# pashtari/factorizer

Hardware: AMD Instinct MI355X
Metric: volumes/sec fwd+bwd, Swin Factorizer 128^3 (higher is better)
Workload: dtype f32

## Files before the change

### factorizer_amd/_native.py

```python
from __future__ import annotations

import ctypes
import os
import threading

import torch

_HERE = os.path.dirname(os.path.abspath(__file__))
LIB_PATH = os.environ.get("FZ_LIB_PATH") or os.path.join(_HERE, "libfactorizer_hip.so")

FZ_OK = 0
FZ_E_UNSUPPORTED = -2
ABI_VERSION = 7
SOLVER_ID = {"mu": 0, "hals": 1, "cd": 2, "smu": 3}
STORE_F32, STORE_BF16 = 0, 1
PRODUCTS_DEFAULT, PRODUCTS_SPLIT_BF16, PRODUCTS_FP32_MFMA = 0, 1, 2
_products = threading.local()


def products() -> int:
    return getattr(_products, "value", PRODUCTS_DEFAULT)


class use_products:
# ... 184 lines not shown
    "fz_gcorr_wgrad": ([_vp] * 4 + [_i] * 11 + [_vp], _i),
    "fz_gcorr_act": ([_vp] * 5 + [_i] * 11 + [_f, _i, _vp], _i),
    "fz_gcorr_wgrad_act": ([_vp] * 4 + [_i] * 12 + [_vp], _i),
    "fz_gcorr_mu_bwd": ([_vp] * 8 + [_i] * 11 + [_f, _i, _vp], _i),
    "fz_gnmf_supported": ([_i, _i64, _i, _i, _i], _i),
    "fz_gnmf_workspace_bytes": ([_i64, _i, _i64, _i, _i, _i], _i64),
    "fz_gnmf_launches": ([_i, _i, _i], _i),
    "fz_gnmf_fwd": ([_vp] * 6 + [_i64, _i, _i64, _i, _i, _i, _f, _vp, _vp], _i),
    "fz_gnmf_bwd": ([_vp] * 7 + [_i64, _i, _i64, _i, _i, _i, _i, _f, _vp, _vp], _i),
    "fz_nmf_cf_supported": ([_i] * 11, _i),
    "fz_nmf_cf_fwd": ([_vp] * 4 + [_i] * 5 + [_c.POINTER(_i)] + [_i] * 5 + [_f, _i, _vp], _i),
    "fz_nmf_cf_bwd": ([_vp] * 5 + [_i] * 5 + [_c.POINTER(_i)] + [_i] * 7 + [_f, _i, _vp], _i),
    "fz_nmf_cf_factors_supported": ([_i] * 12 + [_c.POINTER(_i)], _i),
    "fz_nmf_cf_fwd_store_factors": ([_vp] * 5 + [_i] * 5 + [_c.POINTER(_i)] + [_i] * 3 + [_f, _i, _vp], _i),
    "fz_nmf_cf_fwd_from_factors": ([_vp] * 6 + [_i] * 5 + [_c.POINTER(_i)] * 2 + [_i] * 4 + [_f, _i, _vp], _i),
    "fz_nmf_cf_bwd_factors_supported": ([_i] * 14 + [_c.POINTER(_i)], _i),
    "fz_nmf_cf_bwd_store_factors": ([_vp] * 5 + [_i] * 5 + [_c.POINTER(_i)] + [_i] * 3 + [_f, _i, _vp], _i),
    "fz_nmf_cf_bwd_from_factors": ([_vp] * 6 + [_i] * 5 + [_c.POINTER(_i)] * 2 + [_i] * 3 + [_f, _i, _vp], _i),
    "fz_nmf_pcf_supported": ([_i] * 11, _i),
    "fz_nmf_pcf_fwd": ([_vp] * 4 + [_i] * 8 + [_c.POINTER(_i)] + [_i] * 5 + [_f, _i, _vp], _i),
    "fz_nmf_pcf_bwd": ([_vp] * 5 + [_i] * 8 + [_c.POINTER(_i)] + [_i] * 7 + [_f, _i, _vp], _i),
    "fz_nmf_pcf_bwd_prefers_separate": ([_i] * 4, _i),
    "fz_act_add": ([_vp, _vp, _i64, _i, _vp], _i),
    "fz_mlp_pre_supported": ([_i, _i, _i64, _i], _i),
    "fz_mlp_drop_supported": ([_i, _i, _i64, _i], _i),
    "fz_mlp_chain_drop": ([_c.POINTER(MlpDesc), _c.POINTER(MlpDropout), _vp], _i),
    "fz_conv3_prologue_supported": ([_i] * 4, _i),
    "fz_conv3_fwd2": ([_vp] * 4 + [_i] * 8 + [_c.POINTER(BlockPrologue), _vp], _i),
    "fz_upcat2": ([_vp, _vp, _vp, _i, _vp, _vp, _vp] + [_i] * 7 + [_c.POINTER(BlockPrologue), _vp], _i),
    "fz_gemm": ([_c.POINTER(GemmDesc), _vp], _i),
    "fz_gemm_bx_enable": ([_i], _i),
    "fz_gemm_lnbwd_partials": ([_c.POINTER(GemmDesc)], _i64),
    "fz_reduce_rows": ([_vp, _i64, _i, _vp, _vp, _vp], _i),
    "fz_adamw_step": ([_vp, _vp, _vp, _vp, _i64, _f, _f, _f, _f, _f, _i, _f, _vp], _i),
    "fz_sw_gather": ([_vp, _vp] + [_i] * 10 + [_vp], _i),
    "fz_sw_accumulate": ([_vp] * 6 + [_f] + [_i] * 10 + [_vp], _i),
    "fz_sw_finalize": ([_vp, _vp, _i, _i64, _vp], _i),
    "fz_sw_gather2": ([_vp, _vp] + [_i] * 11 + [_vp], _i),
    "fz_sw_accumulate2": ([_vp] * 6 + [_f] + [_i] * 11 + [_vp], _i),
    "fz_sw_finalize2": ([_vp, _vp, _vp, _i, _i64, _i, _vp], _i),
    "fz_mlp_supported": ([_i, _i, _i64], _i),
    "fz_mlp_partials": ([_i, _i64], _i64),
    "fz_mlp_wgrad_rows": ([_i, _i64], _i),
    "fz_gemm_dw_rows": ([_i, _i64], _i),
    "fz_gemm_dw_workspace_bytes": ([_i, _i64], _i64),
    "fz_gemm_dw": ([_c.POINTER(GemmDwDesc), _vp], _i),
    "fz_mlp_wgrad_workspace_bytes": ([_i, _i64], _i64),
    "fz_mlp_chain": ([_c.POINTER(MlpDesc), _vp], _i),
    "fz_head_bwd_rows": ([], _i),
    "fz_head_bwd_workspace_bytes": ([], _i64),
    "fz_head_bwd": ([_vp, _vp, _vp, _vp, _vp, _i, _i, _i, _i64, _i, _vp], _i),
    "fz_head_fwd": ([_vp, _vp, _vp, _vp, _i, _i, _i, _i64, _i, _vp], _i),
    "fz_upcat_supported": ([_i] * 5, _i),
    "fz_upcat_compose": ([_vp, _vp, _i, _vp, _vp, _vp, _vp, _vp, _i, _i, _i, _vp], _i),
    "fz_upcat_wgrads": ([_vp, _vp, _vp, _i, _vp, _vp, _vp, _vp, _i, _vp, _i, _i, _i, _vp], _i),
    "fz_upcat": ([_vp, _vp, _vp, _i, _vp, _vp, _vp] + [_i] * 7 + [_vp], _i),
    "fz_upcat_bwd_supported": ([_i] * 6, _i),
    "fz_upcat_bwd_workspace_bytes": ([_i] * 4, _i64),
    "fz_upcat_bwd": ([_vp, _vp, _vp, _vp, _i, _vp, _vp, _vp, _vp, _vp, _i, _vp, _vp] + [_i] * 7 + [_vp], _i),
    "fz_wgrad": ([_c.POINTER(WgradDesc), _vp, _vp], _i),
    "fz_wgrad_group": ([_c.POINTER(_c.POINTER(WgradDesc)), _c.POINTER(_vp), _i, _vp], _i),
    "fz_wgrad_workspace_bytes": ([_c.POINTER(WgradDesc)], _i64),
    "fz_conv3_fwd": ([_vp] * 4 + [_i] * 8 + [_vp], _i),
    "fz_conv3_wgrad_chunks": ([_i] * 4, _i),
    "fz_conv3_wgrad_partials": ([_vp] * 4 + [_i] * 8 + [_vp], _i),
    "fz_chunk_reduce": ([_vp, _i, _i64, _vp, _i, _vp], _i),
    "fz_chunk_reduce_ld": ([_vp, _i, _i64, _i64, _vp, _i, _vp], _i),
    "fz_finish_defer": ([_i], _i),
    "fz_finish_pending": ([], _i),
    "fz_finish_flush": ([_vp], _i),
    "fz_finish_flush_all": ([_vp], _i),
    "fz_dice_bce_chunks": ([_i64], _i),
    "fz_dice_bce_sums": ([_vp, _vp, _vp, _i, _i64, _vp], _i),
    "fz_dice_bce_grad": ([_vp, _vp, _vp, _vp, _i, _i64, _f, _f, _vp, _vp], _i),
    "fz_dice_ce_sums": ([_vp, _vp, _vp, _i, _i, _i64, _vp], _i),
    "fz_dice_ce_grad": ([_vp, _vp, _vp, _vp, _i, _i, _i64, _f, _f, _vp, _vp], _i),
    "fz_dice_ce_finish": ([_vp, _i, _i, _i64, _f, _vp, _vp, _vp], _i),
    "fz_dice_bce_ds_sums": ([_vp, _vp, _vp, _i] + [_i] * 6 + [_i, _vp], _i),
    "fz_dice_bce_ds_grad": ([_vp, _vp, _vp, _vp, _i] + [_i] * 6 + [_i, _f, _f, _vp, _vp], _i),
    "fz_dice_ce_ds_sums": ([_vp, _vp, _vp, _i, _i] + [_i] * 6 + [_i, _vp], _i),
    "fz_dice_ce_ds_grad": ([_vp, _vp, _vp, _vp, _i, _i] + [_i] * 6 + [_i, _f, _f, _vp, _vp], _i),
    "fz_rowsum_chunks": ([_i64], _i),
    "fz_rowsum": ([_vp, _vp, _vp, _i, _i, _i64, _i, _vp], _i),
    "fz_ln_fwd": ([_vp] * 5 + [_i, _i, _i64, _f, _i, _vp], _i),
    "fz_ln_bwd": ([_vp] * 8 + [_i, _i, _i64, _i, _vp], _i),
    "fz_ln_bwd_workspace_bytes": ([_i], _i64),
    "fz_ln_bwd_workspace_bytes2": ([_i, _i, _i64], _i64),
    "fz_dropout_bits_words": ([_i, _i, _i64], _i64),
    "fz_dropout_keep_bits": ([_vp, _i, _i, _i, _i64, _f, _vp, _vp], _i),
    "fz_dropout_apply": ([_i, _vp, _f, _vp, _vp, _vp, _i, _i, _i64, _i, _vp], _i),
    "fz_seg_counts_chunks": ([_i64], _i),
    "fz_seg_counts_workspace_bytes": ([_i, _i64], _i64),
    "fz_seg_counts": ([_vp, _i, _vp, _i, _f, _vp, _vp, _vp, _i, _i64, _vp], _i),
    "fz_mask_edges": ([_vp, _vp, _vp, _i, _i, _i, _i, _i, _vp], _i),
    "fz_edge_min_dist2_splits": ([_i64, _i64], _i),
    "fz_edge_min_dist2_workspace_bytes": ([_i64, _i64], _i64),
    "fz_edge_min_dist2": ([_vp, _i64, _vp, _i64, _f, _f, _f, _vp, _vp, _vp], _i),
    "fz_aug_record_floats": ([], _i),
    "fz_aug_resample": ([_vp, _vp, _i, _i, _vp, _vp, _i, _vp, _vp, _vp] + [_i] * 6 + [_vp], _i),
    "fz_aug_smooth": ([_vp, _vp, _i, _i, _vp, _vp] + [_i] * 6 + [_vp], _i),
    "fz_aug_noise_field": ([_vp, _vp, _i, _i, _i64, _vp], _i),
    "fz_aug_source_words": ([], _i),
    "fz_aug_crop_resample": ([_vp, _vp, _i, _i, _vp, _i, _vp, _vp, _vp] + [_i] * 6 + [_vp], _i),
    "fz_vol_kind_ok": ([_i, _i], _i),
    "fz_vol_bbox": ([_vp, _i, _i, _i, _i, _i, _i, _vp, _vp], _i),
    "fz_vol_workspace_bytes": ([_i, _c.POINTER(VolGeom)], _i64),
# ... 18 lines not shown
```

### factorizer_amd/blocks.py

```python
from __future__ import annotations

import os

import torch
from torch import nn

from . import functional as Fn
from . import pointwise as PW
from .layers import MLP, LayerNorm, Linear
from .matricize import Matricize, SWMatricize
from .nmf import NMF, MatrixFactorization, RandomInit
from .utils import partialize


def _env_int(name, default):
    v = os.environ.get(name)
    if v is None:
        return default
    try:
        return int(v, 0)
    except ValueError:
        raise ValueError(f"{name}={v!r}: expected an integer") from None


# ... 37 lines not shown
        self.mlp = MLP(channels, ratio=mlp_ratio, dropout=dropout)

    def _fusable(self, x) -> bool:
        f, m = self.fact, self.mlp
        if not (x.is_cuda and x.numel() and x.dtype in (torch.float32, torch.bfloat16) and PW._vox(x) % 4 == 0
                and x.shape[1] % 2 == 0):
            return False
        if any(p.dtype != torch.float32 for p in self.parameters()):
            return False
        if not (isinstance(self.norm1, LayerNorm) and isinstance(self.norm2, LayerNorm)
                and self.norm1.norm.elementwise_affine and self.norm2.norm.elementwise_affine
                and self.norm1.norm.bias is not None and self.norm2.norm.bias is not None):
            return False
        if not (isinstance(f.act, nn.ReLU) and isinstance(f.in_proj, Linear) and isinstance(f.out_proj, Linear)):
            return False
        blk = m.block
        if not (len(blk) == 5 and isinstance(blk[1], nn.GELU) and blk[1].approximate == "none"
                and blk[0].linear.weight.shape[0] % 2 == 0):
            return False
        drops = (f.dropout, blk[2], blk[4])
        if self.training and any(d.p > 0 for d in drops):
            return all(type(d) is nn.Dropout and 0 <= d.p < 1 for d in drops)
        return True

    def _dropout_ps(self):
        ps = (float(self.fact.dropout.p), float(self.mlp.block[2].p), float(self.mlp.block[4].p))
        return ps if self.training and any(p > 0 for p in ps) else None

    def _modular_native_cfg(self, x) -> bool:
        f = self.fact
        mf = f.factorize
        if not (isinstance(f.reshape, SWMatricize) and isinstance(mf, MatrixFactorization)):
            return False
        t_like = x.new_empty((1, *f.reshape.output_size[1:]))
        return mf._native_solver(t_like) is not None and not mf._wide and len(f.reshape.geometry.spatial) <= 3

    def _core_cfg(self):
        f = self.fact
        mf = f.factorize
        if not (isinstance(f.reshape, SWMatricize) and isinstance(mf, MatrixFactorization)):
            return None
        sid = getattr(mf.solver, "native_id", None)
        if sid is None or not isinstance(mf.init, RandomInit) or mf.solver.factor != (0, 1) or mf.verbose:
            return None
        G = min(max(mf.num_grad_steps, 0), mf.num_iters)
        geo = f.reshape.geometry
        if tuple(mf.size) != (8, geo.P) or not Fn.nmf_core_supported(geo, mf.rank, mf.num_iters, G):
            return None
        return G, sid

    def prologue_params(self, like):
        f, blk = self.fact, self.mlp.block
        n1 = self.norm1.norm
        if not (like.is_cuda and like.shape[1] == 32 and self._fusable(like) and self._core_cfg() is not None
                and f.in_proj.linear.bias is None and blk[0].linear.bias is not None and blk[3].linear.bias is not None
                and f.out_proj.linear.bias is not None and f.in_proj.linear.weight.dtype == torch.float32
                and n1.weight is not None and n1.bias is not None
                and not (self.norm1._forward_hooks or f.in_proj._forward_hooks or f._forward_hooks)):
            return None
        return n1.weight, n1.bias, n1.eps, f.in_proj.linear.weight

    def forward(self, x):
        if self._fusable(x):
            f, blk = self.fact, self.mlp.block
            n1, n2 = self.norm1.norm, self.norm2.norm
            core = self._core_cfg()
            mf = f.factorize
            nat = core is not None or self._modular_native_cfg(x)
            drop = self._dropout_ps()
            one_node = nat and f.in_proj.linear.bias is None and blk[0].linear.bias is not None \
                and blk[3].linear.bias is not None and f.out_proj.linear.bias is not None
            if one_node:
                if core is not None:
                    G, sid = core
                else:
                    G, sid = min(max(mf.num_grad_steps, 0), mf.num_iters), mf.solver.native_id
                cfg = dict(geo=f.reshape.geometry, T=mf.num_iters, G=G, solver=sid, nmf_eps=mf.solver.eps,
                           eps1=n1.eps, eps2=n2.eps, core=core is not None)
                if drop is not None:
                    cfg["drop"] = drop
                args = (x, n1.weight, n1.bias, f.in_proj.linear.weight, mf.init.u0, mf.init.v0,
                        f.out_proj.linear.weight, f.out_proj.linear.bias, n2.weight, n2.bias,
                        blk[0].linear.weight, blk[0].linear.bias, blk[3].linear.weight, blk[3].linear.bias, cfg)
                pre = PW.BlockPrologue.take(x) if core is not None else None
                t_pre, st_pre = pre if pre is not None else (None, None)
                slot = PW.head_fusion_slot()
                if slot is not None and slot.block is self and core is not None and drop is None:
                    hw, hb = slot.head_params
                    C, Hd = x.shape[1], blk[0].linear.weight.shape[0]
                    if PW.block_head_fusable(C, Hd, x[0, 0].numel(), hw, x):
                        y, raw = PW.FactorizerBlockFn.apply(*args, hw, hb, t_pre, st_pre)
                        slot.logits = PW.HeadOfBlockFn.apply(y, hw, hb, raw)
                        return y
                return PW.FactorizerBlockFn.apply(*args, None, None, t_pre, st_pre)
            if drop is None:
                return self._per_layer(x)
        x = x + self.fact(self.norm1(x))
        x = x + self.mlp(self.norm2(x))
        return x

    def _per_layer(self, x):
        f, blk = self.fact, self.mlp.block
        n1, n2 = self.norm1.norm, self.norm2.norm
        t = PW.ln_linear(x, n1.weight, n1.bias, n1.eps, f.in_proj.linear.weight, f.in_proj.linear.bias, "relu")
        a = f.reshape.inverse_forward(f.factorize(f.reshape(t)))
        x = PW.act_linear_res(a, f.out_proj.linear.weight, f.out_proj.linear.bias, x, "none")
        z = PW.ln_linear(x, n2.weight, n2.bias, n2.eps, blk[0].linear.weight, blk[0].linear.bias, "none")
# ... 66 lines not shown
```

### factorizer_amd/csrc/upcat.hip

```cpp
#include "gemm_bx.h"
#include "finish.h"

namespace fz {

template <typename AT>
struct UpcatArgsT {
  const AT* skip;
  const AT* deep;
  const float* wa;
  const float* wbt;
  const float* bias;
  AT* out;
  int lda;
  int B, D, H, W;
  BlockPrologueArgs pro;
};

#ifndef UPCAT_WAVES
#define UPCAT_WAVES 4
#endif
#define UPCAT_THREADS (UPCAT_WAVES * 64)
template <typename AT, bool PRO = false>
__global__ __launch_bounds__(UPCAT_THREADS, 1) void upcat_bx_kernel(UpcatArgsT<AT> p, unsigned ntiles) {
  constexpr int C = 32, CD = 64;
// ... 177 lines not shown
  if (tile + tstep < ntiles) fetch(tile + tstep, xsB, xdB);
  for (; tile < ntiles; tile += 2 * tstep) {
    run(tile, xsA, xdA);
    if (tile + tstep < ntiles) run(tile + tstep, xsB, xdB);
  }
}

__global__ __launch_bounds__(256) void upcat_compose_kernel(const float* __restrict__ w_t, const float* __restrict__ w_b, int ldb,
                                                            const float* __restrict__ b_t, const float* __restrict__ b_ad,
                                                            float* __restrict__ wc, float* __restrict__ wbt,
                                                            float* __restrict__ bias, int Cd, int O, int M) {
  const int k = blockIdx.x;
  if (k == Cd) {
    if (bias == nullptr) return;
    for (int m = threadIdx.x; m < M; m += 256) {
      float t = b_ad != nullptr ? b_ad[m] : 0.f;
      if (b_t != nullptr)
        for (int c = 0; c < O; ++c) t += w_b[(int64_t)m * ldb + c] * b_t[c];
      bias[m] = t;
    }
    return;
  }
  const float* wk = w_t + (int64_t)k * O * 8;
  for (int i = threadIdx.x; i < M * 8; i += 256) {
    const int m = i >> 3, t = i & 7;
    float acc = 0.f;
    for (int c = 0; c < O; ++c) acc += wk[c * 8 + t] * w_b[(int64_t)m * ldb + c];
    if (wc != nullptr) wc[((int64_t)k * M + m) * 8 + t] = acc;
    if (wbt != nullptr) wbt[((int64_t)t * M + m) * Cd + k] = acc;
  }
}


}

using namespace fz;

extern "C" int fz_upcat_compose(const float* w_t, const float* w_b, int ldb, const float* b_t, const float* b_ad, float* wc, float* wbt,
                                float* bias, int Cd, int O, int M, fz_stream_t stream) {
  if (!w_t || !w_b || (!wc && !wbt && !bias) || Cd < 1 || O < 1 || M < 1 || ldb < O) return fail(FZ_E_ARG, "fz_upcat_compose: bad arguments");
  hipLaunchKernelGGL(upcat_compose_kernel, dim3((unsigned)(Cd + 1)), dim3(256), 0, (hipStream_t)stream, w_t, w_b, ldb, b_t, b_ad, wc, wbt,
                     bias, Cd, O, M);
  FZ_LAUNCH_CHECK();
  return FZ_OK;
}

extern "C" int fz_upcat_wgrads(const float* gt, const float* w_t, const float* w_b, int ldb, const float* gb_ad, const float* b_t,
                               float* gw_t, float* gw_b, int ldg, float* gb_t, int Cd, int O, int M, fz_stream_t stream) {
  if (!gt || !w_t || !w_b || !gb_ad || !gw_t || !gw_b || Cd < 1 || O < 1 || M < 1 || ldb < O || ldg < O)
    return fail(FZ_E_ARG, "fz_upcat_wgrads: bad arguments");
  FinishJob fj = finish_job(FK_UPCAT, fin_upcat_blocks(Cd, O, M), 1);
  fj.u.up = FinUpcat{gt, w_t, w_b, gb_ad, b_t, gw_t, gw_b, gb_t, ldb, ldg, Cd, O, M};
  return finish_run(&fj, 1, (hipStream_t)stream);
}

extern "C" int fz_upcat_supported(int C, int Cd, int D, int H, int W) {
  return C == 32 && Cd == 64 && D >= 1 && H >= 1 && W >= 1 && (2 * W) % 64 == 0 && ((int64_t)2 * H * 2 * W) % 256 == 0 &&
         (int64_t)64 * D * H * W * 8 * 4 < ((int64_t)1 << 31);
}

template <typename AT>
static int upcat_launch(const void* skip, const void* deep, const float* wa, int lda, const float* wbt, const float* bias, void* out,
                        int B, int D, int H, int W, const fz_block_prologue* pro, fz_stream_t stream) {
  UpcatArgsT<AT> a;
  a.pro = BlockPrologueArgs{};
  if (pro) a.pro = BlockPrologueArgs{pro->ln_g, pro->ln_b, pro->ln_eps, pro->w, pro->t, pro->stats};
  a.skip = (const AT*)skip; a.deep = (const AT*)deep; a.wa = wa; a.wbt = wbt; a.bias = bias; a.out = (AT*)out;
  a.lda = lda; a.B = B; a.D = D; a.H = H; a.W = W;
  const int64_t ntiles = (int64_t)8 * D * H * W / 64 * B;
  if (ntiles >= ((int64_t)1 << 30)) return fail(FZ_E_ARG, "fz_upcat: more than 2^30 wave tiles (32-bit tile arithmetic)");
  constexpr int lds = (2 + 8 * 4) * 3 * 64 * 16 + 2 * 3 * 64 * 16 + 32 * 4;
  const int64_t wgs = (ntiles + UPCAT_WAVES - 1) / UPCAT_WAVES;
  if (pro) {
    auto kern = upcat_bx_kernel<AT, true>;
    FZ_HIP_OK(hipFuncSetAttribute(reinterpret_cast<const void*>(kern), hipFuncAttributeMaxDynamicSharedMemorySize, lds));
    hipLaunchKernelGGL(kern, dim3((unsigned)(wgs < 256 ? wgs : 256)), dim3(UPCAT_THREADS), lds, (hipStream_t)stream, a, (unsigned)ntiles);
    FZ_LAUNCH_CHECK();
    return FZ_OK;
  }
  auto kern = upcat_bx_kernel<AT>;
  FZ_HIP_OK(hipFuncSetAttribute(reinterpret_cast<const void*>(kern), hipFuncAttributeMaxDynamicSharedMemorySize, lds));
  hipLaunchKernelGGL(kern, dim3((unsigned)(wgs < 256 ? wgs : 256)), dim3(UPCAT_THREADS), lds, (hipStream_t)stream, a, (unsigned)ntiles);
  FZ_LAUNCH_CHECK();
  return FZ_OK;
}

extern "C" int fz_upcat2(const void* skip, const void* deep, const float* wa, int lda, const float* wbt, const float* bias, void* out,
                         int B, int C, int Cd, int D, int H, int W, int act_dtype, const fz_block_prologue* pro, fz_stream_t stream) {
  if (!skip || !deep || !wa || !wbt || !out) return fail(FZ_E_ARG, "fz_upcat: null pointer");
  if (pro && (!pro->ln_g || !pro->ln_b || !pro->w || !pro->t || !pro->stats)) return fail(FZ_E_ARG, "fz_upcat2: incomplete block prologue");
  if (!fz_upcat_supported(C, Cd, D, H, W) || lda < C) return fail(FZ_E_UNSUPPORTED, "fz_upcat: needs C = 32, 64 deep channels, 2W % 64 == 0, 4HW % 256 == 0");
  if (B <= 0) return B == 0 ? FZ_OK : fail(FZ_E_SHAPE, "fz_upcat: negative batch");
  if (act_dtype == FZ_STORE_F32) return upcat_launch<float>(skip, deep, wa, lda, wbt, bias, out, B, D, H, W, pro, stream);
  if (act_dtype == FZ_STORE_BF16) return upcat_launch<bf16>(skip, deep, wa, lda, wbt, bias, out, B, D, H, W, pro, stream);
  return fail(FZ_E_ARG, "fz_upcat: act_dtype must be FZ_STORE_F32 or FZ_STORE_BF16");
}

extern "C" int fz_upcat(const void* skip, const void* deep, const float* wa, int lda, const float* wbt, const float* bias, void* out,
                        int B, int C, int Cd, int D, int H, int W, int act_dtype, fz_stream_t stream) {
  return fz_upcat2(skip, deep, wa, lda, wbt, bias, out, B, C, Cd, D, H, W, act_dtype, nullptr, stream);
}
```

### factorizer_amd/pointwise.py

```python
from __future__ import annotations

import collections
import ctypes
import os
import threading as _threading
import weakref

import torch
import torch.nn.functional as F

from . import _native as N
from . import gradbuf as _GB
from . import functional as Fn

ACT = {"none": 0, "relu": 1, "gelu": 2}
LOAD_PLAIN, LOAD_S2D, LOAD_K3, LOAD_S2D_2D, LOAD_K3_2D = 0, 1, 2, 3, 4
EPI_PLAIN, EPI_D2S, EPI_D2S_2D = 0, 1, 3
QL_S2D_2D, QL_K3_2D = LOAD_S2D_2D, LOAD_K3_2D
_D2S_FINE = {EPI_D2S: 8, EPI_D2S_2D: 4}


def _p(t):
    return None if t is None else t.data_ptr()

# ... 995 lines not shown
    y = torch.matmul(weight.reshape(weight.shape[0], weight.shape[1]), x.reshape(B, C, _vox(x)))
    if bias is not None:
        y = y + bias.view(1, -1, 1)
    return y.reshape(B, weight.shape[0], *x.shape[2:])


def layernorm_cf(x, weight, bias, eps):
    if weight is not None and bias is not None and _native_ok(x, weight, bias):
        return LayerNormFn.apply(x, weight, bias, eps)
    _warn_composed("LayerNorm", x, weight, bias)
    y = F.layer_norm(x.movedim(1, -1), (x.shape[1],), weight, bias, eps)
    return y.movedim(-1, 1).contiguous()


def mlp_cf(x, w1, b1, w2, b2):
    if _native_ok(x, w1, b1, w2, b2) and w1.shape[1] % 2 == 0 and w2.shape[1] % 2 == 0:
        z = LinearFn.apply(x, w1, b1)
        return ActLinearResFn.apply(z, w2, b2, None, "gelu")
    _warn_composed("MLP", x, w1, b1, w2, b2)
    return linear_cf(F.gelu(linear_cf(x, w1, b1)), w2, b2)


def ln_linear(x, ln_w, ln_b, eps, w, b, act="none"):
    if _native_ok(x, ln_w, ln_b, w, b) and w.shape[1] % 2 == 0:
        return LNLinearFn.apply(x, ln_w, ln_b, eps, w, b, act)
    _warn_composed("LayerNorm+Linear", x, ln_w, ln_b, w, b)
    y = linear_cf(layernorm_cf(x, ln_w, ln_b, eps), w, b)
    return torch.relu(y) if act != "none" else y


def act_linear_res(z, w, b, res, act="none"):
    if _native_ok(z, w, b, res) and w.shape[1] % 2 == 0:
        return ActLinearResFn.apply(z, w, b, res, act)
    _warn_composed("Linear+residual", z, w, b, res)
    y = linear_cf(F.gelu(z) if act == "gelu" else z, w, b)
    return y if res is None else res + y


class UpCatLinearFn(torch.autograd.Function):

    _fz_acts = (0, 1, 6)

    @staticmethod
    @_fwd
    def forward(ctx, skip, deep, w_t, b_t, w_ad, b_ad, pro=None):
        skip, deep = skip.contiguous(), deep.contiguous()
        B, Cd, D, H, W = deep.shape
        O = w_t.shape[1]
        V = D * H * W
        C1 = skip.shape[1]
        M = w_ad.shape[0]
        w2 = w_ad.reshape(M, C1 + O)
        y = torch.empty((B, M, *skip.shape[2:]), dtype=skip.dtype, device=skip.device)
        if (M == 32 and C1 == 32 and O == 32 and _UPCAT_FWD and N.lib().fz_upcat_supported(C1, Cd, D, H, W)):
            w_b = w2[:, C1:]
            wbt = torch.empty((8, M, Cd), dtype=torch.float32, device=skip.device)
            bias = torch.empty(M, dtype=torch.float32, device=skip.device) if (b_t is not None or b_ad is not None) else None
            with torch.cuda.device(skip.device):
                N.check(N.lib().fz_upcat_compose(w_t.data_ptr(), w_b.data_ptr(), C1 + O, _p(b_t), _p(b_ad), None, wbt.data_ptr(),
                                                 _p(bias), Cd, O, M, N.stream_ptr(skip)), "fz_upcat_compose")
            es = skip.element_size()
            bp = None
            if pro is not None:
                ln_w, ln_b, eps, w_in = pro
                t_pro = torch.empty_like(y)
                st_pro = torch.empty((B, 2, 8 * V), dtype=torch.float32, device=skip.device)
                bp = N.BlockPrologue(ln_w.data_ptr(), ln_b.data_ptr(), float(eps), w_in.data_ptr(), t_pro.data_ptr(), st_pro.data_ptr())
            with torch.cuda.device(skip.device):
                rc = Fn._timed(f"upcat_{Cd}->{M}" + ("_ln_linear" if bp is not None else ""),
                               es * (skip.numel() + deep.numel() + y.numel() * (2 if bp is not None else 1)),
                               lambda: N.lib().fz_upcat2(skip.data_ptr(), deep.data_ptr(), w2.data_ptr(), C1 + O, wbt.data_ptr(),
                                                         _p(bias), y.data_ptr(), B, C1, Cd, D, H, W, N.act_dtype(skip),
                                                         ctypes.byref(bp) if bp is not None else None, N.stream_ptr(skip)),
                               cols=B * 8 * V, flops=2 * B * 8 * V * M * (C1 + Cd))
            N.check(rc, "fz_upcat")
        elif pro is not None:
            raise RuntimeError("UpCatLinearFn: a block prologue needs the one-pass forward (callers check upcat_prologue_ok)")
        else:
            up = torch.empty((B, O, 2 * D, 2 * H, 2 * W), dtype=deep.dtype, device=deep.device)
            _gemm([deep], w_t, up, B=B, Cin=Cd, Vin=V, M=8 * O, K=Cd, Ncol=V, w_t=True, ldw=8 * O, bias=b_t,
                  epilogue=EPI_D2S, Ho=H, Wo=W, name="tconv_k2s2")
            _gemm([skip, up], w2, y, B=B, Cin=C1 + O, Vin=8 * V, M=M, K=C1 + O, Ncol=8 * V, bias=b_ad, c0=C1, name="cat_linear")
        ctx.save_for_backward(skip, deep, w_t, w2, b_t)
        ctx.has_bt, ctx.has_bad, ctx.wshape = b_t is not None, b_ad is not None, w_ad.shape
        ctx.npro = 0 if pro is None else 1
        if pro is not None:
            ctx.mark_non_differentiable(t_pro, st_pro)
            ctx.set_materialize_grads(False)
            return y, t_pro, st_pro
        return y

    @staticmethod
    def _backward_three(ctx, g, skip, deep, w2, wc, gw_ad, gb_ad, gt):
        B, Cd, D, H, W = deep.shape
        V = D * H * W
        Vf = 8 * V
        C1 = skip.shape[1]
        M = w2.shape[0]
        O = w2.shape[1] - C1
        dev = g.device
        if M == 32 and C1 == 32 and _dw_fused_ok(M, Vf):
            g_skip, _, _, _, _ = _gemm_dw(g, w2[:, :C1], skip, want_bias=True, name="dgrad_wgrad",
                                          gw_out=gw_ad[:, :C1], gb_out=gb_ad)
        else:
            g_skip = torch.empty_like(skip)
            _gemm([g], w2, g_skip, B=B, Cin=M, Vin=Vf, M=C1, K=M, Ncol=Vf, w_t=True, ldw=C1 + O, name="linear_dgrad")
            gwa = torch.empty((M, C1), dtype=torch.float32, device=dev)
# ... 23 lines not shown
        C1 = skip.shape[1]
        M = w2.shape[0]
        dev = g.device
        gw_ad = _GB.out_like(w2)
        gb_ad = torch.empty(M, dtype=torch.float32, device=dev)
        w_b = w2[:, C1:]
        wc = torch.empty((Cd, M, 2, 2, 2), dtype=torch.float32, device=dev)
        with torch.cuda.device(dev):
            N.check(N.lib().fz_upcat_compose(w_t.data_ptr(), w_b.data_ptr(), C1 + O, None, None, wc.data_ptr(), None, None,
                                             Cd, O, M, N.stream_ptr(g)), "fz_upcat_compose")
        gt = torch.empty((Cd, M, 8), dtype=torch.float32, device=dev)
        if (M == 32 and ctx.needs_input_grad[1] and _UPCAT_BWD and skip.dtype == g.dtype == deep.dtype
                and N.lib().fz_upcat_bwd_supported(C1, Cd, D, H, W, N.act_dtype(g))
                and not ((g.data_ptr() | skip.data_ptr()) & 7 or deep.data_ptr() & 15)):
            g_skip, g_deep = torch.empty_like(skip), torch.empty_like(deep)
            ws = torch.empty(N.lib().fz_upcat_bwd_workspace_bytes(B, D, H, W) // 4, dtype=torch.float32, device=dev)
            es = g.element_size()
            with torch.cuda.device(dev), _finish_scope(ws, gt, gw_ad, gb_ad):
                rc = Fn._timed(f"upcat_bwd_{Cd}->{M}", es * (3 * g.numel() + 2 * deep.numel()),
                               lambda: N.lib().fz_upcat_bwd(g.data_ptr(), skip.data_ptr(), deep.data_ptr(), w2.data_ptr(), C1 + O,
                                                            wc.data_ptr(), g_skip.data_ptr(), g_deep.data_ptr(), ws.data_ptr(),
                                                            gw_ad.data_ptr(), C1 + O, gb_ad.data_ptr(), gt.data_ptr(), B, C1, Cd,
                                                            D, H, W, N.act_dtype(g), N.stream_ptr(g)),
                               cols=B * Vf, flops=4 * B * Vf * M * (C1 + Cd))
            N.check(rc, "fz_upcat_bwd")
        else:
            g_skip, g_deep = UpCatLinearFn._backward_three(ctx, g, skip, deep, w2, wc, gw_ad, gb_ad, gt)
        gw_t = _GB.out_like(w_t)
        gb_t = torch.empty(O, dtype=torch.float32, device=dev) if ctx.has_bt else None
        with torch.cuda.device(dev), _finish_scope(gt, gb_ad, gw_t, gw_ad, gb_t):
            N.check(N.lib().fz_upcat_wgrads(gt.data_ptr(), w_t.data_ptr(), w_b.data_ptr(), C1 + O, gb_ad.data_ptr(), _p(b_t),
                                            gw_t.data_ptr(), gw_ad[:, C1:].data_ptr(), C1 + O, _p(gb_t), Cd, O, M,
                                            N.stream_ptr(g)), "fz_upcat_wgrads")
        return (g_skip, g_deep, gw_t, gb_t, gw_ad.reshape(ctx.wshape), gb_ad if ctx.has_bad else None, None)[:len(ctx.needs_input_grad)]


_UPCAT_FWD = os.environ.get("FZ_UPCAT_FWD", "1") != "0"
_UPCAT_BWD = os.environ.get("FZ_UPCAT_BWD", "1") != "0"
_HEAD_BWD = os.environ.get("FZ_HEAD_BWD", "1") != "0"


def up_cat_linear(skip, deep, w_t, b_t, w_ad, b_ad=None, pro=None):
    return UpCatLinearFn.apply(skip, deep, w_t, b_t, w_ad, b_ad, pro)


_PRODUCER_PROLOGUE = os.environ.get("FZ_PRODUCER_PROLOGUE", "1") != "0"


def conv3_prologue_ok(x, w):
    return (_PRODUCER_PROLOGUE and x.is_cuda and x.dim() == 5 and x.shape[1] * 27 * 64 * 4 <= 65536 and x.dtype in (torch.float32, torch.bfloat16)
            and bool(N.lib().fz_conv3_prologue_supported(int(x.shape[1]), int(w.shape[0]), int(x.shape[-1]), N.products())))


def upcat_prologue_ok(skip, deep, w_t, w_ad):
    B, Cd, D, H, W = deep.shape
    O, C1, M = w_t.shape[1], skip.shape[1], w_ad.shape[0]
    return (_PRODUCER_PROLOGUE and M == 32 and C1 == 32 and O == 32 and _UPCAT_FWD and bool(N.lib().fz_upcat_supported(C1, Cd, D, H, W)))


class BlockPrologue:
    _tls = _threading.local()

    def __init__(self, x, t, st):
        self.x, self.t, self.st = x, t, st

    def __enter__(self):
        tls = BlockPrologue._tls
        self.prev = getattr(tls, "cur", None)
        tls.cur = self
        return self

    def __exit__(self, *exc):
        BlockPrologue._tls.cur = self.prev

    @staticmethod
    def take(x):
        cur = getattr(BlockPrologue._tls, "cur", None)
        if cur is not None and cur.x is x:
            return cur.t, cur.st
        return None


def cat_linear(x1, x2, w, b=None):
    if _native_ok(x1, x2, w, b) and x1.shape[1] % 2 == 0 and x2.shape[1] % 2 == 0:
        return CatLinearFn.apply(x1, x2, w, b)
    _warn_composed("cat+Linear", x1, x2, w, b)
    return linear_cf(torch.cat([x1, x2], dim=1), w, b)


def _block_dropout_bits(x, C, Hd, drop):
    B, V = x.shape[0], _vox(x)
    seed = Fn.dropout_seed(x.device)
    return tuple(None if p == 0 else Fn.dropout_keep_bits(seed, s, B, ch, V, p) for s, (ch, p) in enumerate(zip((C, Hd, C), drop)))


def _block_dropout_fwd(a, wout2, bout, x, ln_w, ln_b, eps, w12, b1, w22, b2, drop, bits):
    B, C = x.shape[:2]
    V = _vox(x)
    Hd = w12.shape[0]
    new = lambda ch: torch.empty((B, ch, *x.shape[2:]), dtype=x.dtype, device=x.device)
    (p0, p1, p2), (m0, m1, m2) = drop, bits
    if m0 is not None:
        o = new(C)
        _gemm([a], wout2, o, B=B, Cin=C, Vin=V, M=C, K=C, Ncol=V, bias=bout, name="linear")
        x1 = Fn.dropout_apply(N.DROP_RES, m0, p0, o, x)
        del o
    else:
        x1 = new(C)
        _gemm([a], wout2, x1, B=B, Cin=C, Vin=V, M=C, K=C, Ncol=V, bias=bout, res=x, name="act_linear_res")
    z1 = new(Hd)
# ... 298 lines not shown
```

### include/factorizer_hip.h

```cpp
#ifndef FACTORIZER_HIP_H
#define FACTORIZER_HIP_H

#include <stdint.h>

#ifdef __cplusplus
extern "C" {
#endif

#define FZ_OK 0
#define FZ_E_SHAPE (-1)
#define FZ_E_UNSUPPORTED (-2)
#define FZ_E_HIP (-3)
#define FZ_E_ARG (-4)

#define FZ_STORE_F32 0
#define FZ_STORE_BF16 1

#define FZ_SOLVER_MU 0
#define FZ_SOLVER_HALS 1
#define FZ_SOLVER_CD 2
#define FZ_SOLVER_SMU 3

typedef void* fz_stream_t;

// ... 167 lines not shown
  const float* pre_b;
  const void* pre_res;
  void* pre_out;
  const float* post_w;
  const float* post_b;
  void* post_out;
  int post_m;
} fz_mlp_desc;
typedef struct fz_mlp_dropout {
  const uint32_t* m0;
  const uint32_t* m1;
  const uint32_t* m2;
  float s0, s1, s2;
} fz_mlp_dropout;

typedef struct fz_gemm_dw_desc {
  const void* g;
  const void* q;
  const float* w;
  int ln;
  const float* stats;
  const float* ln_g;
  const float* ln_b;
  const void* gadd;
  void* y;
  float* gln;
  void* wpart;
  float* gw;
  float* gb;
  int B, C;
  int64_t V;
  int act_dtype;
  int ldgw;
  int ldw;
  const uint32_t* drop_m;
  float drop_s;
} fz_gemm_dw_desc;
int fz_gemm_dw_rows(int B, int64_t V);
int64_t fz_gemm_dw_workspace_bytes(int B, int64_t V);
int fz_gemm_dw(const fz_gemm_dw_desc* desc, fz_stream_t stream);

int fz_head_bwd_rows(void);
int64_t fz_head_bwd_workspace_bytes(void);
int fz_head_bwd(const void* gy, const void* x, const float* w, void* gx, float* part, int B, int M, int C, int64_t V,
                int act_dtype, fz_stream_t stream);
int fz_head_fwd(const void* x, const float* w, const float* bias, void* y, int B, int M, int C, int64_t V, int act_dtype,
                fz_stream_t stream);

int fz_upcat_compose(const float* w_t, const float* w_b, int ldb, const float* b_t, const float* b_ad, float* wc, float* wbt, float* bias,
                     int Cd, int O, int M, fz_stream_t stream);
int fz_upcat_wgrads(const float* gt, const float* w_t, const float* w_b, int ldb, const float* gb_ad, const float* b_t, float* gw_t,
                    float* gw_b, int ldg, float* gb_t, int Cd, int O, int M, fz_stream_t stream);
int fz_upcat_supported(int C, int Cd, int D, int H, int W);
int fz_upcat(const void* skip, const void* deep, const float* wa, int lda, const float* wbt, const float* bias, void* out,
             int B, int C, int Cd, int D, int H, int W, int act_dtype, fz_stream_t stream);
int fz_upcat_bwd_supported(int C1, int Cd, int D, int H, int W, int act_dtype);
int64_t fz_upcat_bwd_workspace_bytes(int B, int D, int H, int W);
int fz_upcat_bwd(const void* g, const void* skip, const void* deep, const float* wa, int lda, const float* wc, void* g_skip,
                 void* g_deep, void* workspace, float* gw_a, int ldg, float* gb, float* gt, int B, int C1, int Cd, int D, int H,
                 int W, int act_dtype, fz_stream_t stream);
typedef struct fz_block_prologue {
  const float* ln_g;
  const float* ln_b;
  float ln_eps;
  const float* w;
  void* t;
  float* stats;
} fz_block_prologue;
int fz_upcat2(const void* skip, const void* deep, const float* wa, int lda, const float* wbt, const float* bias, void* out,
              int B, int C, int Cd, int D, int H, int W, int act_dtype, const fz_block_prologue* pro, fz_stream_t stream);

int fz_mlp_supported(int C, int H, int64_t V);
int fz_mlp_pre_supported(int C, int H, int64_t V, int products);
int fz_mlp_drop_supported(int C, int H, int64_t V, int products);
int64_t fz_mlp_partials(int B, int64_t V);
int fz_mlp_wgrad_rows(int B, int64_t V);
int64_t fz_mlp_wgrad_workspace_bytes(int B, int64_t V);
int fz_mlp_chain(const fz_mlp_desc* desc, fz_stream_t stream);
int fz_mlp_chain_drop(const fz_mlp_desc* desc, const fz_mlp_dropout* drop, fz_stream_t stream);

#define FZ_QL_PLAIN 0
#define FZ_QL_S2D 1
#define FZ_QL_K3 2
#define FZ_QL_S2D_2D 3
#define FZ_QL_K3_2D 4

typedef struct fz_wgrad_desc {
  const void* p;
  int M;
  const void* pmul;
  int pmul_kind;
  const void* q[4];
  int nsrc, src_mode, c0;
  int Cin;
  int K;
  int64_t Vq;
  int D, H, W;
  int64_t N;
  int Ho, Wo;
  const float* stats;
  int qact;
  const float* ln_g;
  const float* ln_b;
  float* gw;
  float* gbias;
  int accumulate;
// ... 180 lines not shown
```

Baseline: 131.2.

## Add fused upcat kernel for 64-channel decoder stage with block prologue

Adds a new HIP kernel that fuses the transposed-conv upsample, concat and 1x1 projection for the C=64/Cd=128 decoder level in fp32, using split-bf16 MFMA. It optionally also fuses the next block's LayerNorm plus in-projection and ReLU, writing the normalization stats. The Python dispatch and the prologue eligibility check are widened to accept 64 channels, so this level no longer falls back to separate unfused ops. In exchange it adds a large specialized kernel with heavy register and LDS use, plus a three-term bf16 split approximation of fp32 products.

```diff
diff --git a/factorizer_amd/_native.py b/factorizer_amd/_native.py
--- a/factorizer_amd/_native.py
+++ b/factorizer_amd/_native.py
@@ -260,6 +260,7 @@
     "fz_head_bwd": ([_vp, _vp, _vp, _vp, _vp, _i, _i, _i, _i64, _i, _vp], _i),
     "fz_head_fwd": ([_vp, _vp, _vp, _vp, _i, _i, _i, _i64, _i, _vp], _i),
     "fz_upcat_supported": ([_i] * 5, _i),
+    "fz_upcat_fwd_supported": ([_i] * 6, _i),
     "fz_upcat_compose": ([_vp, _vp, _i, _vp, _vp, _vp, _vp, _vp, _i, _i, _i, _vp], _i),
     "fz_upcat_wgrads": ([_vp, _vp, _vp, _i, _vp, _vp, _vp, _vp, _i, _vp, _i, _i, _i, _vp], _i),
     "fz_upcat": ([_vp, _vp, _vp, _i, _vp, _vp, _vp] + [_i] * 7 + [_vp], _i),
diff --git a/factorizer_amd/blocks.py b/factorizer_amd/blocks.py
--- a/factorizer_amd/blocks.py
+++ b/factorizer_amd/blocks.py
@@ -113,7 +113,7 @@
     def prologue_params(self, like):
         f, blk = self.fact, self.mlp.block
         n1 = self.norm1.norm
-        if not (like.is_cuda and like.shape[1] == 32 and self._fusable(like) and self._core_cfg() is not None
+        if not (like.is_cuda and like.shape[1] in (32, 64) and self._fusable(like) and self._core_cfg() is not None
                 and f.in_proj.linear.bias is None and blk[0].linear.bias is not None and blk[3].linear.bias is not None
                 and f.out_proj.linear.bias is not None and f.in_proj.linear.weight.dtype == torch.float32
                 and n1.weight is not None and n1.bias is not None
diff --git a/factorizer_amd/csrc/upcat.hip b/factorizer_amd/csrc/upcat.hip
--- a/factorizer_amd/csrc/upcat.hip
+++ b/factorizer_amd/csrc/upcat.hip
@@ -253,6 +253,17 @@
   FinishJob fj = finish_job(FK_UPCAT, fin_upcat_blocks(Cd, O, M), 1);
   fj.u.up = FinUpcat{gt, w_t, w_b, gb_ad, b_t, gw_t, gw_b, gb_t, ldb, ldg, Cd, O, M};
   return finish_run(&fj, 1, (hipStream_t)stream);
+}
+
+namespace fz {
+int upcat64_supported(int C, int Cd, int D, int H, int W, int act_dtype);
+int upcat64_launch(const void* skip, const void* deep, const float* wa, int lda, const float* wbt, const float* bias, void* out, int B,
+                   int D, int H, int W, const fz_block_prologue* pro, fz_stream_t stream);
+}
+
+extern "C" int fz_upcat_fwd_supported(int C, int Cd, int D, int H, int W, int act_dtype) {
+  if (act_dtype != FZ_STORE_F32 && act_dtype != FZ_STORE_BF16) return 0;
+  return fz_upcat_supported(C, Cd, D, H, W) || upcat64_supported(C, Cd, D, H, W, act_dtype);
 }
 
 extern "C" int fz_upcat_supported(int C, int Cd, int D, int H, int W) {
@@ -290,7 +301,14 @@
                          int B, int C, int Cd, int D, int H, int W, int act_dtype, const fz_block_prologue* pro, fz_stream_t stream) {
   if (!skip || !deep || !wa || !wbt || !out) return fail(FZ_E_ARG, "fz_upcat: null pointer");
   if (pro && (!pro->ln_g || !pro->ln_b || !pro->w || !pro->t || !pro->stats)) return fail(FZ_E_ARG, "fz_upcat2: incomplete block prologue");
-  if (!fz_upcat_supported(C, Cd, D, H, W) || lda < C) return fail(FZ_E_UNSUPPORTED, "fz_upcat: needs C = 32, 64 deep channels, 2W % 64 == 0, 4HW % 256 == 0");
+  if (upcat64_supported(C, Cd, D, H, W, act_dtype) && lda >= C) {
+    if (B <= 0) return B == 0 ? FZ_OK : fail(FZ_E_SHAPE, "fz_upcat: negative batch");
+    if (((uintptr_t)skip | (uintptr_t)out | (pro ? (uintptr_t)pro->t | (uintptr_t)pro->stats : 0)) & 7)
+      return fail(FZ_E_ARG, "fz_upcat: skip, out, t and stats must be 8-byte aligned");
+    return upcat64_launch(skip, deep, wa, lda, wbt, bias, out, B, D, H, W, pro, stream);
+  }
+  if (!fz_upcat_supported(C, Cd, D, H, W) || lda < C)
+    return fail(FZ_E_UNSUPPORTED, "fz_upcat: needs C = 32 with 64 deep channels, 2W % 64 == 0, 4HW % 256 == 0, or C = 64 with 128 in fp32 storage, 2W % 64 == 0");
   if (B <= 0) return B == 0 ? FZ_OK : fail(FZ_E_SHAPE, "fz_upcat: negative batch");
   if (act_dtype == FZ_STORE_F32) return upcat_launch<float>(skip, deep, wa, lda, wbt, bias, out, B, D, H, W, pro, stream);
   if (act_dtype == FZ_STORE_BF16) return upcat_launch<bf16>(skip, deep, wa, lda, wbt, bias, out, B, D, H, W, pro, stream);
diff --git a/factorizer_amd/csrc/upcat64.hip b/factorizer_amd/csrc/upcat64.hip
--- /dev/null
+++ b/factorizer_amd/csrc/upcat64.hip
@@ -0,0 +1,328 @@
+#include "gemm_bx.h"
+
+namespace fz {
+
+struct Upcat64Args {
+  const float* skip;
+  const float* deep;
+  const float* wa;
+  const float* wbt;
+  const float* bias;
+  float* out;
+  int lda;
+  int B, D, H, W;
+  BlockPrologueArgs pro;
+};
+
+constexpr int kU64SlotF = 3 * 256;
+constexpr int kU64SlotsMain = 8 + 32;
+constexpr int kU64LdsMain = kU64SlotsMain * kU64SlotF * 4 + 64 * 4;
+constexpr int kU64LdsPro = (kU64SlotsMain + 8) * kU64SlotF * 4 + 128 * 4;
+
+template <bool PRO>
+__global__ __launch_bounds__(256, 1) void upcat64_kernel(Upcat64Args p, unsigned ntc, unsigned S) {
+  constexpr int C = 64, CD = 128, M = 64;
+  constexpr int GS = C / 16, GD = CD / 16;
+  extern __shared__ __attribute__((aligned(16))) float As[];
+  const int lane = threadIdx.x & 63;
+  const int wave = __builtin_amdgcn_readfirstlane((int)(threadIdx.x >> 6));
+  const int j = lane & 31, hk = lane >> 5;
+  const unsigned nw = gridDim.x >> 2, bid = blockIdx.x;
+  const bool xcd = (nw & 7u) == 0;
+  const unsigned cls = xcd ? (bid >> 3) & 3u : bid & 3u, wi = xcd ? (bid & 7u) + 8u * (bid >> 5) : bid >> 2;
+  const unsigned td = cls >> 1, th = cls & 1u;
+  const unsigned Wf = 2u * p.W, Hf = 2u * p.H;
+  const int64_t Vc = (int64_t)p.D * p.H * p.W, Vf = 8 * Vc;
+  const unsigned rows_per_sample = (unsigned)p.D * (unsigned)p.H;
+
+#pragma unroll
+  for (int it = 0; it < kU64SlotsMain * 64 / 256; ++it) {
+    const int item = it * 256 + (int)threadIdx.x;
+    const int l = item & 63, slot = item >> 6;
+    const int kh = l >> 5;
+    float a8[8];
+    if (slot < 8) {
+      const int mb = slot >> 2, g = slot & 3;
+      const float* src = p.wa + (int64_t)(32 * mb + (l & 31)) * p.lda + 16 * g + 8 * kh;
+#pragma unroll
+      for (int e = 0; e < 8; ++e) a8[e] = src[e];
+    } else {
+      const int s2 = slot - 8, q = s2 >> 4, mb = (s2 >> 3) & 1, g = s2 & 7;
+      const int tap = (int)cls * 2 + q;
+      const float* src = p.wbt + ((int64_t)tap * M + 32 * mb + (l & 31)) * CD + 16 * g + 8 * kh;
+#pragma unroll
+      for (int e = 0; e < 8; ++e) a8[e] = src[e];
+    }
+    bx8 t3[3];
+    bx_split<3>(a8, t3);
+    bx8* dst = reinterpret_cast<bx8*>(As) + (slot * 3) * 64 + l;
+    dst[0] = t3[0]; dst[64] = t3[1]; dst[128] = t3[2];
+  }
+  float* sbias = As + (PRO ? kU64SlotsMain + 8 : kU64SlotsMain) * kU64SlotF;
+  float* twp = sbias + 64;
+  if (threadIdx.x < 64) sbias[threadIdx.x] = p.bias != nullptr ? p.bias[threadIdx.x] : 0.f;
+  if constexpr (PRO) {
+#pragma unroll
+    for (int it = 0; it < 2; ++it) {
+      const int item = it * 256 + (int)threadIdx.x;
+      const int l = item & 63, s = item >> 6;
+      const int mo = s >> 2, G = s & 3, mbk = G >> 1, g = G & 1;
+      float wv[8];
+#pragma unroll
+      for (int e = 0; e < 8; ++e) {
+        const int r = 8 * g + e;
+        const int kk = 32 * mbk + (r & 3) + 8 * (r >> 2) + 4 * (l >> 5);
+        wv[e] = p.pro.w[(32 * mo + (l & 31)) * 64 + kk] * p.pro.ln_g[kk];
+      }
+      bx8 t3[3];
+      bx_split<3>(wv, t3);
+      bx8* dst = reinterpret_cast<bx8*>(As) + ((kU64SlotsMain + s) * 3) * 64 + l;
+      dst[0] = t3[0]; dst[64] = t3[1]; dst[128] = t3[2];
+    }
+    {
+      const int row = threadIdx.x >> 2, part = threadIdx.x & 3;
+      float s = 0.f;
+#pragma unroll
+      for (int k = 0; k < 16; ++k) s += p.pro.w[row * 64 + 16 * part + k] * p.pro.ln_b[16 * part + k];
+      s += __shfl_xor(s, 1, 64);
+      s += __shfl_xor(s, 2, 64);
+      if (part == 0) twp[row] = s;
+    }
+  }
+  __syncthreads();
+
+  struct Tile { unsigned b, n0, nc0; };
+  auto locate = [&](unsigned u) {
+    const unsigned row = u / S, s = u - row * S;
+    const unsigned b = row / rows_per_sample, rr = row - b * rows_per_sample;
+    const unsigned dz = rr / (unsigned)p.H, hy = rr - dz * (unsigned)p.H;
+    Tile t;
+    t.b = b;
+    t.n0 = ((2u * dz + td) * Hf + 2u * hy + th) * Wf + 64u * s;
+    t.nc0 = rr * (unsigned)p.W + 32u * s;
+    return t;
+  };
+
+  typedef float XsT[GS][8][2];
+  typedef float XdT[GD][8];
+  auto fetch_skip = [&](const Tile& t, XsT& xs) {
+    const unsigned soff = (unsigned)((((int64_t)8 * hk) * Vf + t.n0 + 2 * j) * 4);
+#pragma unroll
+    for (int g = 0; g < GS; ++g) {
+      const float* ub = p.skip + ((int64_t)t.b * C + 16 * g) * Vf;
+#pragma unroll
+      for (int e = 0; e < 8; ++e) uload<2>(ub + (int64_t)e * Vf, soff, xs[g][e]);
+    }
+  };
+  auto fetch_deep = [&](const Tile& t, XdT& xd, int g0) {
+    const unsigned doff = (unsigned)((((int64_t)8 * hk) * Vc + t.nc0 + j) * 4);
+#pragma unroll
+    for (int g = g0; g < g0 + GD / 2; ++g) {
+      const float* ub = p.deep + ((int64_t)t.b * CD + 16 * g) * Vc;
+#pragma unroll
+      for (int e = 0; e < 8; ++e) {
+        float t1[1];
+        uload<1>(ub + (int64_t)e * Vc, doff, t1);
+        xd[g][e] = t1[0];
+      }
+    }
+  };
+
+  const unsigned ustep = nw * 4u;
+  auto run = [&](unsigned u, XsT& xs, XdT& xd, XsT& xsn, XdT& xdn) {
+    const bool more = u + ustep < ntc;
+    const Tile tl = locate(u), tn = locate(more ? u + ustep : u);
+    if (more) fetch_skip(tn, xsn);
+    __builtin_amdgcn_sched_barrier(0);
+    int lane4 = lane * 4;
+    asm volatile("" : "+v"(lane4));
+    const float* Al = As + lane4;
+
+    f32x16 acc[2][2];
+#pragma unroll
+    for (int mb = 0; mb < 2; ++mb)
+#pragma unroll
+      for (int q = 0; q < 2; ++q)
+#pragma unroll
+        for (int r = 0; r < 16; ++r) acc[mb][q][r] = 0.f;
+    auto slot_of = [](int st, int mb) { return st < 4 ? mb * 4 + st : 8 + (((st - 4) & 1) * 2 + mb) * 8 + ((st - 4) >> 1); };
+    auto load_a = [&](int st, bx8 (&a)[6]) {
+#pragma unroll
+      for (int mb = 0; mb < 2; ++mb)
+#pragma unroll
+        for (int t = 0; t < 3; ++t) a[mb * 3 + t] = *reinterpret_cast<const bx8*>(Al + (slot_of(st, mb) * 3 + t) * 256);
+    };
+    bx8 aop[2][6], bd[3];
+    load_a(0, aop[0]);
+#pragma unroll
+    for (int st = 0; st < GS + 2 * GD; ++st) {
+      if (st == GS || st == GS + GD) {
+        __builtin_amdgcn_sched_barrier(0);
+        if (more) fetch_deep(tn, xdn, st == GS ? 0 : GD / 2);
+        __builtin_amdgcn_sched_barrier(0);
+      }
+      if (st + 1 < GS + 2 * GD) load_a(st + 1, aop[(st + 1) & 1]);
+      if (st < GS) {
+        bx8 bs[2][3];
+#pragma unroll
+        for (int q = 0; q < 2; ++q) {
+          float x8[8];
+#pragma unroll
+          for (int e = 0; e < 8; ++e) x8[e] = xs[st][e][q];
+          bx_split<3>(x8, bs[q]);
+        }
+#pragma unroll
+        for (int mb = 0; mb < 2; ++mb)
+#pragma unroll
+          for (int t = 2; t >= 0; --t)
+#pragma unroll
+            for (int q = 0; q < 2; ++q)
+#pragma unroll
+              for (int jj = 2; jj >= 0; --jj)
+                if (t + jj <= 2) acc[mb][q] = __builtin_amdgcn_mfma_f32_32x32x16_bf16(aop[st & 1][mb * 3 + t], bs[q][jj], acc[mb][q], 0, 0, 0);
+      } else {
+        const int g = (st - GS) >> 1, q = (st - GS) & 1;
+        if (q == 0) bx_split<3>(xd[g], bd);
+#pragma unroll
+        for (int mb = 0; mb < 2; ++mb)
+#pragma unroll
+          for (int t = 2; t >= 0; --t)
+#pragma unroll
+            for (int jj = 2; jj >= 0; --jj)
+              if (t + jj <= 2) acc[mb][q] = __builtin_amdgcn_mfma_f32_32x32x16_bf16(aop[st & 1][mb * 3 + t], bd[jj], acc[mb][q], 0, 0, 0);
+      }
+    }
+
+    const unsigned yoff = (unsigned)((((int64_t)4 * hk) * Vf + tl.n0 + 2 * j) * 4);
+    float* yb = p.out + (int64_t)tl.b * M * Vf;
+    float yv[2][2][16];
+#pragma unroll
+    for (int mb = 0; mb < 2; ++mb)
+#pragma unroll
+      for (int r = 0; r < 16; ++r) {
+        const int rb = 32 * mb + (r & 3) + 8 * (r >> 2);
+        const float add = sbias[rb + 4 * hk];
+        const float v[2] = {acc[mb][0][r] + add, acc[mb][1][r] + add};
+        vstore<2>(reinterpret_cast<float*>(reinterpret_cast<char*>(yb + (int64_t)rb * Vf) + yoff), v);
+        if constexpr (PRO) { yv[0][mb][r] = v[0]; yv[1][mb][r] = v[1]; }
+      }
+    if constexpr (PRO) {
+      float mu[2], rs[2];
+#pragma unroll
+      for (int q = 0; q < 2; ++q) {
+        float s = 0.f;
+#pragma unroll
+        for (int i = 0; i < 32; ++i) s += yv[q][i >> 4][i & 15];
+        s += __shfl_xor(s, 32, 64);
+        mu[q] = s / 64.0f;
+        float v = 0.f;
+#pragma unroll
+        for (int i = 0; i < 32; ++i) {
+          const float d = yv[q][i >> 4][i & 15] - mu[q];
+          v += d * d;
+        }
+        v += __shfl_xor(v, 32, 64);
+        rs[q] = 1.0f / sqrtf(v / 64.0f + p.pro.ln_eps);
+#pragma unroll
+        for (int i = 0; i < 32; ++i) yv[q][i >> 4][i & 15] = (yv[q][i >> 4][i & 15] - mu[q]) * rs[q];
+      }
+      f32x16 tacc[2][2];
+#pragma unroll
+      for (int mo = 0; mo < 2; ++mo)
+#pragma unroll
+        for (int q = 0; q < 2; ++q)
+#pragma unroll
+          for (int r = 0; r < 16; ++r) tacc[mo][q][r] = 0.f;
+      bx8 wop[2][6];
+      auto load_w = [&](int G, bx8 (&a)[6]) {
+#pragma unroll
+        for (int mo = 0; mo < 2; ++mo)
+#pragma unroll
+          for (int t = 0; t < 3; ++t) a[mo * 3 + t] = *reinterpret_cast<const bx8*>(Al + ((kU64SlotsMain + mo * 4 + G) * 3 + t) * 256);
+      };
+      load_w(0, wop[0]);
+#pragma unroll
+      for (int G = 0; G < 4; ++G) {
+        if (G + 1 < 4) load_w(G + 1, wop[(G + 1) & 1]);
+        bx8 bop[2][3];
+#pragma unroll
+        for (int q = 0; q < 2; ++q) {
+          float x8[8];
+#pragma unroll
+          for (int e = 0; e < 8; ++e) x8[e] = yv[q][G >> 1][8 * (G & 1) + e];
+          bx_split<3>(x8, bop[q]);
+        }
+#pragma unroll
+        for (int mo = 0; mo < 2; ++mo)
+#pragma unroll
+          for (int t = 2; t >= 0; --t)
+#pragma unroll
+            for (int q = 0; q < 2; ++q)
+#pragma unroll
+              for (int jj = 2; jj >= 0; --jj)
+                if (t + jj <= 2) tacc[mo][q] = __builtin_amdgcn_mfma_f32_32x32x16_bf16(wop[G & 1][mo * 3 + t], bop[q][jj], tacc[mo][q], 0, 0, 0);
+      }
+      float* tb = reinterpret_cast<float*>(p.pro.t) + (int64_t)tl.b * M * Vf;
+#pragma unroll
+      for (int mo = 0; mo < 2; ++mo)
+#pragma unroll
+        for (int r = 0; r < 16; ++r) {
+          const int rb = 32 * mo + (r & 3) + 8 * (r >> 2);
+          const float add = twp[rb + 4 * hk];
+          const float v[2] = {fmaxf(tacc[mo][0][r] + add, 0.f), fmaxf(tacc[mo][1][r] + add, 0.f)};
+          vstore<2>(reinterpret_cast<float*>(reinterpret_cast<char*>(tb + (int64_t)rb * Vf) + yoff), v);
+        }
+      if (hk == 0) {
+        float* so = p.pro.stats + (int64_t)tl.b * 2 * Vf + tl.n0 + 2 * j;
+        *reinterpret_cast<float2*>(so) = make_float2(mu[0], mu[1]);
+        *reinterpret_cast<float2*>(so + Vf) = make_float2(rs[0], rs[1]);
+      }
+    }
+  };
+
+  XsT xsA, xsB;
+  XdT xdA, xdB;
+  unsigned u = wi * 4u + (unsigned)wave;
+  if (u < ntc) {
+    const Tile t0 = locate(u);
+    fetch_skip(t0, xsA);
+    fetch_deep(t0, xdA, 0);
+    fetch_deep(t0, xdA, GD / 2);
+  }
+  for (; u < ntc; u += 2 * ustep) {
+    run(u, xsA, xdA, xsB, xdB);
+    if (u + ustep < ntc) run(u + ustep, xsB, xdB, xsA, xdA);
+  }
+}
+
+int upcat64_supported(int C, int Cd, int D, int H, int W, int act_dtype) {
+  return C == 64 && Cd == 128 && act_dtype == FZ_STORE_F32 && D >= 1 && H >= 1 && W >= 1 && (2 * W) % 64 == 0 &&
+         (int64_t)64 * D * H * W * 8 * 4 < ((int64_t)1 << 31);
+}
+
+int upcat64_launch(const void* skip, const void* deep, const float* wa, int lda, const float* wbt, const float* bias, void* out, int B,
+                   int D, int H, int W, const fz_block_prologue* pro, fz_stream_t stream) {
+  Upcat64Args a;
+  a.pro = BlockPrologueArgs{};
+  if (pro) a.pro = BlockPrologueArgs{pro->ln_g, pro->ln_b, pro->ln_eps, pro->w, pro->t, pro->stats};
+  a.skip = (const float*)skip; a.deep = (const float*)deep; a.wa = wa; a.wbt = wbt; a.bias = bias; a.out = (float*)out;
+  a.lda = lda; a.B = B; a.D = D; a.H = H; a.W = W;
+  const unsigned S = (unsigned)(2 * W / 64);
+  const int64_t ntc = (int64_t)B * D * H * S;
+  if (ntc >= ((int64_t)1 << 30)) return fail(FZ_E_ARG, "fz_upcat: more than 2^30 wave tiles per class (32-bit tile arithmetic)");
+  const int64_t wgc = (ntc + 3) / 4;
+  const dim3 grid((unsigned)(4 * (wgc < 64 ? wgc : 64)));
+  if (pro) {
+    auto kern = upcat64_kernel<true>;
+    FZ_HIP_OK(hipFuncSetAttribute(reinterpret_cast<const void*>(kern), hipFuncAttributeMaxDynamicSharedMemorySize, kU64LdsPro));
+    hipLaunchKernelGGL(kern, grid, dim3(256), kU64LdsPro, (hipStream_t)stream, a, (unsigned)ntc, S);
+  } else {
+    auto kern = upcat64_kernel<false>;
+    FZ_HIP_OK(hipFuncSetAttribute(reinterpret_cast<const void*>(kern), hipFuncAttributeMaxDynamicSharedMemorySize, kU64LdsMain));
+    hipLaunchKernelGGL(kern, grid, dim3(256), kU64LdsMain, (hipStream_t)stream, a, (unsigned)ntc, S);
+  }
+  FZ_LAUNCH_CHECK();
+  return FZ_OK;
+}
+
+}
diff --git a/factorizer_amd/pointwise.py b/factorizer_amd/pointwise.py
--- a/factorizer_amd/pointwise.py
+++ b/factorizer_amd/pointwise.py
@@ -1071,7 +1071,7 @@
         M = w_ad.shape[0]
         w2 = w_ad.reshape(M, C1 + O)
         y = torch.empty((B, M, *skip.shape[2:]), dtype=skip.dtype, device=skip.device)
-        if (M == 32 and C1 == 32 and O == 32 and _UPCAT_FWD and N.lib().fz_upcat_supported(C1, Cd, D, H, W)):
+        if _upcat_fwd_ok(skip, deep, M, O):
             w_b = w2[:, C1:]
             wbt = torch.empty((8, M, Cd), dtype=torch.float32, device=skip.device)
             bias = torch.empty(M, dtype=torch.float32, device=skip.device) if (b_t is not None or b_ad is not None) else None
@@ -1201,10 +1201,15 @@
             and bool(N.lib().fz_conv3_prologue_supported(int(x.shape[1]), int(w.shape[0]), int(x.shape[-1]), N.products())))
 
 
+def _upcat_fwd_ok(skip, deep, M, O):
+    B, Cd, D, H, W = deep.shape
+    C1 = skip.shape[1]
+    return (_UPCAT_FWD and M == C1 == O and skip.dtype == deep.dtype and skip.dtype in (torch.float32, torch.bfloat16)
+            and bool(N.lib().fz_upcat_fwd_supported(C1, Cd, D, H, W, N.act_dtype(skip))))
+
+
 def upcat_prologue_ok(skip, deep, w_t, w_ad):
-    B, Cd, D, H, W = deep.shape
-    O, C1, M = w_t.shape[1], skip.shape[1], w_ad.shape[0]
-    return (_PRODUCER_PROLOGUE and M == 32 and C1 == 32 and O == 32 and _UPCAT_FWD and bool(N.lib().fz_upcat_supported(C1, Cd, D, H, W)))
+    return _PRODUCER_PROLOGUE and _upcat_fwd_ok(skip, deep, w_ad.shape[0], w_t.shape[1])
 
 
 class BlockPrologue:
diff --git a/include/factorizer_hip.h b/include/factorizer_hip.h
--- a/include/factorizer_hip.h
+++ b/include/factorizer_hip.h
@@ -243,6 +243,7 @@
 int fz_upcat_wgrads(const float* gt, const float* w_t, const float* w_b, int ldb, const float* gb_ad, const float* b_t, float* gw_t,
                     float* gw_b, int ldg, float* gb_t, int Cd, int O, int M, fz_stream_t stream);
 int fz_upcat_supported(int C, int Cd, int D, int H, int W);
+int fz_upcat_fwd_supported(int C, int Cd, int D, int H, int W, int act_dtype);
 int fz_upcat(const void* skip, const void* deep, const float* wa, int lda, const float* wbt, const float* bias, void* out,
              int B, int C, int Cd, int D, int H, int W, int act_dtype, fz_stream_t stream);
 int fz_upcat_bwd_supported(int C1, int Cd, int D, int H, int W, int act_dtype);
```

After: 132.0, median of 6. No clear change (+0.6%).
